# wkvong/multimodal-baby

Hardware: AMD Instinct MI355X
Metric: image-text pairs/sec, CVCL ResNeXt+embed 224², bs256, 1/2/4/8 MI355X (higher is better)
Workload: dtype bf16; 1 GPU; C2 = BASELINE configs[1]: CVCL saycam_contrastive, frozen random-init ResNeXt-50 32x4d (BN train mode) + embedding mean-pool text encoder, E=512, L2-normalised, fixed tau 0.07, 224x224 frames + 3-word utterances; full step = fwd + InfoNCE + bwd(fc, embedding) + AdamW; per_gpu_batch=256, global_batch=256, negatives=local (single GPU), parallelism=dp1, trunk_streams=2

## Files before the change

### include/cvcl_hip.h

```cpp
#ifndef CVCL_HIP_H
#define CVCL_HIP_H

#include <stddef.h>
#include <stdint.h>

#ifdef __cplusplus
extern "C" {
#endif

#define CVCL_ABI_VERSION 7

enum { CVCL_OK = 0, CVCL_EINVAL = -1, CVCL_ELAUNCH = -2, CVCL_EWORKSPACE = -3, CVCL_EUNSUPPORTED = -4 };
enum { CVCL_F32 = 0, CVCL_BF16 = 1, CVCL_F32X3 = 2 };
enum { CVCL_ACT_NONE = 0, CVCL_ACT_RELU = 1, CVCL_ACT_GELU = 2 };
#define CVCL_STATS_ACCUMULATE (-1)

int cvcl_abi_version(void);
const char* cvcl_last_error(void);

enum { CVCL_K_GEMM = 0, CVCL_K_GCONV = 1, CVCL_K_STEM = 2, CVCL_K_BN_FINALIZE = 3, CVCL_K_BN_ADD_RELU = 4,
       CVCL_K_MAXPOOL = 5, CVCL_K_AVGPOOL = 6, CVCL_K_HEAD = 7, CVCL_K_OTHER = 8, CVCL_K_ATTENTION = 9,
       CVCL_K_LAYERNORM = 10, CVCL_K_LSTM = 11, CVCL_K_GEMM_F32 = 12, CVCL_K_BN_APPLY = 13, CVCL_K_BN_BWD = 14,
       CVCL_K_WGRAD = 15, CVCL_K_GEMM8W = 16, CVCL_K_GEMM_PRO = 17, CVCL_K_NCLASSES = 18 };
int cvcl_prof_enable(int on);
// ... 48 lines not shown
int cvcl_gemm(int dtype, const cvcl_gemm_args* args, void* stream);
int cvcl_gemm_stats_rows(int dtype, const cvcl_gemm_args* args);
int cvcl_gemm8w(int epi, const cvcl_gemm_args* args, void* stream);
int cvcl_gemm_pro(const cvcl_gemm_args* args, void* stream);
int cvcl_gemm_pro_supported(const cvcl_gemm_args* args);
int cvcl_gemm_pro_stats_rows(int M, int N);
int cvcl_gemm8w_supported(int M, int N, int K, int lda, int ldw, int ldc);
int cvcl_set_gemm_cu_share(int cus);
int cvcl_gemm_ln_supported(const cvcl_gemm_args* args);
int cvcl_row_stats(int dtype, const void* x, long x_row_stride, float* out, long rows, int D, float eps, void* stream);
int cvcl_row_stats_finalize(const float* row_part, int strips, float* out, long rows, int D, float eps, void* stream);
int cvcl_gemm8w_tile_rows(int M, int N);
int cvcl_gemm8w_stats_rows(int M, int N);

size_t cvcl_conv1x1_gram_workspace_bytes(int K);
int cvcl_conv1x1_gram(const void* A, int lda, long M, int K, const float* a_scale, const float* a_shift, int a_relu, void* workspace,
                      size_t workspace_bytes, const double** gram_out, void* stream);
int cvcl_bn_from_gram(const double* gram, int K, long count, const void* W, int ldw, int N, const float* gamma, const float* beta,
                      float* running_mean, float* running_var, int64_t* num_batches_tracked, float momentum, float eps,
                      float* scale, float* shift, float* moments, int moments_ld, const float* centre, void* stream);

int cvcl_transpose_f32(const float* in, float* out, int rows, int cols, void* stream);
int cvcl_colsum_f32(const float* dY, float* d_bias, int M, int N, void* stream);

enum { CVCL_PACK_DENSE = 0, CVCL_PACK_STEM7 = 1, CVCL_PACK_GCONV3 = 2 };

typedef struct {
    const void* w;
    const float* gamma; const float* beta;
    float* running_mean; float* running_var; int64_t* num_batches_tracked;
} cvcl_convbn_params;

int cvcl_bn_finalize(const float* stats, int rows, long count, const float* gamma, const float* beta,
                     float* running_mean, float* running_var, int64_t* num_batches_tracked, float momentum,
                     float eps, float* scale, float* shift, const float* centre, int C, void* stream);
int cvcl_bn_eval_affine(const float* gamma, const float* beta, const float* running_mean, const float* running_var,
                        float eps, float* scale, float* shift, const float* centre, int C, void* stream);
int cvcl_col_stats_rows(long rows);
int cvcl_col_stats(int dtype, const void* x, long rows, int C, float* stats, int stats_rows, void* stream);

size_t cvcl_packed_weight_bytes(int dtype, int kind, int cout, int cin_per_group, int k);
int cvcl_pack_conv_weight(int dtype, int kind, const float* w_oihw, void* out, int cout, int cin_per_group, int k,
                          void* stream);

int cvcl_stem_conv_stats_rows(int dtype, int B, int H, int W);
int cvcl_stem_conv7x7(int dtype, const float* x_nchw, const void* w_packed, void* y_nhwc, float* stats, int stats_rows,
                      const float* centre , int B, int H, int W, void* stream);
int cvcl_stem_pool_supported(int dtype, int H, int W);
int cvcl_stem_pool(int dtype, const float* x_nchw, const void* w_packed, const float* scale, const float* shift,
                   const float* centre , void* y_nhwc, int B, int H, int W, void* stream);
int cvcl_bn_relu_maxpool(int dtype, const void* x, const float* scale, const float* shift, void* y, int B, int H, int W,
                         int C, void* stream);
int cvcl_gconv3x3_stats_rows(int dtype, int B, int H, int W, int C, int stride);
int cvcl_gconv3x3(int dtype, const void* x, const float* a_scale, const float* a_shift, const void* w_packed, void* y,
                  float* stats, int stats_rows, const float* centre , int B, int H, int W, int C, int groups,
                  int stride, void* stream);
int cvcl_bn_add_relu(int dtype, const void* raw, const float* scale, const float* shift, const void* idn,
                     const float* idn_scale, const float* idn_shift, void* out, long rows, int C, void* stream);
int cvcl_bn_relu_apply(int dtype, const void* x, const float* scale, const float* shift, void* y, long rows, int C,
                       void* stream);
int cvcl_avgpool(int dtype, const void* x, float* out, int B, int HW, int C, void* stream);

size_t cvcl_resnext50_workspace_bytes(int dtype, int B, int H, int W);
size_t cvcl_resnext50_centres_floats(void);
int cvcl_resnext50_fwd(int dtype, int B, int H, int W, int training, const float* x_nchw,
                       const cvcl_convbn_params* layers, int n_layers, void* workspace, size_t workspace_bytes,
                       void* layer4_out_nhwc, float* pooled, float momentum, float eps, const float* centres, void* stream);
size_t cvcl_resnext50_block_workspace_bytes(int dtype, int B, int h, int w, int stage);
int cvcl_resnext50_block_fwd(int dtype, int B, int h, int w, int stage, int first, int training, const void* x_nhwc,
                             const cvcl_convbn_params* layers, int n_layers, void* workspace, size_t workspace_bytes,
                             void* out_nhwc, float momentum, float eps, const float* centres ,
                             void* stream);
size_t cvcl_resnext50_moments_floats(void);
int cvcl_resnext50_fwd_deferred_stats(int dtype, int B, int H, int W, const float* x_nchw,
                                      const cvcl_convbn_params* layers, int n_layers, void* workspace, size_t workspace_bytes,
                                      void* layer4_out_nhwc, float* pooled, float eps, float* moments, const float* centres,
                                      void* stream);
int cvcl_resnext50_apply_moments(const cvcl_convbn_params* layers, int n_layers, const float* moments, float momentum,
                                 void* stream);
size_t cvcl_resnext50_fwd_grouped_workspace_bytes(int dtype, int B, int H, int W, int group);
int cvcl_resnext50_fwd_grouped(int dtype, int B, int H, int W, int group, const float* x_nchw,
                               const cvcl_convbn_params* layers, int n_layers, void* workspace, size_t workspace_bytes,
                               void* layer4_out_nhwc, float* pooled, float eps, void* stream);

int cvcl_im2col_patches(int dtype, const float* x_nchw, void* cols, int B, int H, int W, int patch, int Kpad,
                        void* stream);
int cvcl_vit_assemble_tokens(int dtype, const void* tok, const float* cls, const float* pos, void* h, int B, int T,
                             int D, void* stream);
int cvcl_layernorm(int dtype, const void* x, long x_row_stride, const float* gamma, const float* beta, float eps,
                   void* y, int y_is_f32, long rows, int D, void* stream);
int cvcl_attention(int dtype, const void* qkv, const int64_t* key_tok, void* out, int B, int T, int heads, int head_dim,
                   float scale, void* stream);
int cvcl_attention_mx(const void* qkv, void* out8, void* out_block_scales, int B, int T, int heads, int head_dim, float scale,
                      void* stream);
int cvcl_attention_train(const void* qkv, void* out, float* lse, int B, int T, int heads, int head_dim, float scale, void* stream);
int cvcl_attention_bwd(const void* qkv, const void* o, const void* d_o, const float* lse, void* d_qkv, int B, int T, int heads,
                       int head_dim, float scale, void* stream);
int cvcl_layernorm_bwd_rows_partials(long rows);
int cvcl_layernorm_bwd_rows(const void* x, long x_row_stride, const float* gamma, const void* dy, int dy_is_f32, long dy_row_stride,
                            float eps, const void* add, void* dx, long dx_row_stride, float* partial, long rows, int D, void* stream);
int cvcl_gelu_bf16(const void* u, const void* d_y, void* y, long n, void* stream);
int cvcl_vit_tokens_bwd(const void* dh, void* d_tok, float* d_pos, int B, int T, int D, void* stream);
int cvcl_attention_train_f32(const float* qkv, float* out, float* lse, int B, int T, int heads, int head_dim, float scale, void* stream);
int cvcl_attention_bwd_f32(const float* qkv, const float* o, const float* d_o, const float* lse, float* d_qkv, int B, int T, int heads,
                           int head_dim, float scale, void* stream);
int cvcl_layernorm_bwd_rows_f32(const float* x, long x_row_stride, const float* gamma, const float* dy, long dy_row_stride, float eps,
// ... 161 lines not shown
```

### multimodal-baby_amd/csrc/resnext.hip

```cpp
#include <algorithm>
#include <array>
#include <cstdlib>
#include <type_traits>

#include "cvcl_common.h"

namespace {

constexpr int kMaxStatsRows = 1024;
constexpr size_t kTrunkAccLayer = (size_t)kBnAccRows * 2 * 2048;


__global__ __launch_bounds__(1024) void bn_finalize_kernel(const float* __restrict__ stats, int rows, double count,
                                                           const float* __restrict__ gamma, const float* __restrict__ beta,
                                                           float* __restrict__ running_mean, float* __restrict__ running_var,
                                                           int64_t* __restrict__ nbt, float momentum, float eps,
                                                           float* __restrict__ scale, float* __restrict__ shift, int C,
                                                           float* __restrict__ moments, int moments_ld,
                                                           const float* __restrict__ centre) {
    constexpr int NS = 64, NC = 16;
    __shared__ double ps[NS][NC], pq[NS][NC];
    const int c = threadIdx.x & (NC - 1), sl = threadIdx.x / NC, ch = blockIdx.x * NC + c;
    double s = 0.0, q = 0.0;
    if (ch < C) {
// ... 519 lines not shown
        const int ox = (int)(p % Wo), oq = (int)((p / Wo) % Hq), b = (int)(p / ((long)Wo * Hq));
        const int oy = R * oq;
        float sc[8], sh[8], m[R][8];
#pragma unroll
        for (int e = 0; e < 8; ++e) {
            sc[e] = scale[cc * 8 + e]; sh[e] = shift[cc * 8 + e];
#pragma unroll
            for (int r = 0; r < R; ++r) m[r][e] = 0.f;
        }
        constexpr int EPC = ElemTraits<T>::kPerChunk, NC = 8 / EPC;
        Chunk<T> tap[NTAP][NC];
        const T* src[NTAP];
#pragma unroll
        for (int ky = 0; ky < NR; ++ky)
#pragma unroll
            for (int kx = 0; kx < 3; ++kx) {
                const int yin = min(max(2 * oy - 1 + ky, 0), H - 1);
                const int xin = min(max(2 * ox - 1 + kx, 0), W - 1);
                src[ky * 3 + kx] = x + (((long)b * H + yin) * W + xin) * C + cc * 8;
            }
        __builtin_amdgcn_sched_barrier(0);
#pragma unroll
        for (int t = 0; t < NTAP; ++t)
#pragma unroll
            for (int q = 0; q < NC; ++q) tap[t][q].load(src[t] + q * EPC);
        __builtin_amdgcn_sched_barrier(0);
#pragma unroll
        for (int t = 0; t < NTAP; ++t)
#pragma unroll
            for (int e = 0; e < 8; ++e) {
                const float v = fmaf(tap[t][e / EPC].get(e % EPC), sc[e], sh[e]);
#pragma unroll
                for (int r = 0; r < R; ++r)
                    if (t >= 6 * r && t < 6 * r + 9) m[r][e] = fmaxf(m[r][e], v);
            }
#pragma unroll
        for (int r = 0; r < R; ++r) {
            if (oy + r < Ho) {
                T* dst = y + (((long)b * Ho + oy + r) * Wo + ox) * C + cc * 8;
#pragma unroll
                for (int e = 0; e < 8; ++e) dst[e] = ElemTraits<T>::from_f(m[r][e]);
            }
        }
    }
}

constexpr int GC_CS = 64;
constexpr int GC_PIXB = 144;

struct GconvDev {
    const void* x; const float* a_scale; const float* a_shift; const void* w; void* y; float* stats;
    const float* centre;
    int B, H, W, C, cg, stride, Ho, Wo, TH, bands, rows_in;
    float act_floor;
    BnSrc src;
    int stats_acc;
};

template <bool WIDE, int NPF, int NMT>
__global__ __launch_bounds__(256, WIDE ? 2 : 3) void gconv_mfma_kernel(GconvDev p) {
    extern __shared__ __attribute__((aligned(16))) char smem[];
    const bf16_t* __restrict__ x = (const bf16_t*)p.x;
    bf16_t* __restrict__ y = (bf16_t*)p.y;
    const int tid = threadIdx.x, lane = tid & 63, wave = tid >> 6;
    const int pix = lane & 15, kb = lane >> 4;
    const int slab = blockIdx.y, c0 = slab * GC_CS;
    const int Wp = p.W + 2;
    constexpr bool wide = WIDE;
    constexpr int KS = WIDE ? 9 : 5;
    const int unit = c0 / 16 + wave;
    const bf16_t* wu = (const bf16_t*)p.w + (long)unit * KS * 512;
    bf16x8 wf[KS];
#pragma unroll
    for (int ks = 0; ks < KS; ++ks) wf[ks] = *reinterpret_cast<const bf16x8*>(wu + (ks * 16 + pix) * 32 + kb * 8);
    const int in_ch_off = wide ? ((wave >> 1) * 32 + kb * 8) : (wave * 16 + (kb & 1) * 8);

    const int s_chunk = tid & 7, s_pix0 = tid >> 3;
    f32x2 sc[4], sh[4];
    if (p.src.acc) {
        float* aff = reinterpret_cast<float*>(smem);
        bn_slice_affine<GC_CS>(p.src, c0, blockIdx.x == 0, aff, aff + 64);
#pragma unroll
        for (int e = 0; e < 4; ++e) {
            const int cl = s_chunk * 8 + 2 * e;
            sc[e] = f32x2{aff[cl], aff[cl + 1]};
            sh[e] = f32x2{aff[64 + cl], aff[64 + cl + 1]};
        }
        __syncthreads();
    } else {
#pragma unroll
        for (int e = 0; e < 4; ++e) {
            const int ch = c0 + s_chunk * 8 + 2 * e;
            sc[e] = p.a_scale ? f32x2{p.a_scale[ch], p.a_scale[ch + 1]} : f32x2{1.f, 1.f};
            sh[e] = p.a_scale ? f32x2{p.a_shift[ch], p.a_shift[ch + 1]} : f32x2{0.f, 0.f};
        }
    }
    const bool relu_in = p.act_floor == 0.f;
    f32x2 ssum[2] = {f32x2{0.f, 0.f}, f32x2{0.f, 0.f}}, ssq[2] = {f32x2{0.f, 0.f}, f32x2{0.f, 0.f}};

    const int npix_in = p.rows_in * Wp;
    const int n_out = p.TH * p.Wo, n_mt = cvcl_div_up(n_out, 16);
    int tap_off[KS];
#pragma unroll
    for (int ks = 0; ks < KS; ++ks) {
        int tap = wide ? ks : 2 * ks + (kb >> 1);
        if (tap > 8) tap = 8;
        const int ky = tap / 3, kx = tap - ky * 3;
        tap_off[ks] = (ky * Wp + kx) * GC_PIXB + in_ch_off * 2;
    }
    int mtab[NMT];
#pragma unroll
    for (int mt = 0; mt < NMT; ++mt) {
        const int q = pix + 16 * mt;
        const bool ok = mt < n_mt && q < n_out;
        const int ty = q / p.Wo, ox = q - ty * p.Wo;
        mtab[mt] = ok ? ((((ty * p.stride) * Wp + ox * p.stride) * GC_PIXB) | (ty << 16) | (1 << 24)) : 0;
    }
    char* s_out = smem + npix_in * GC_PIXB;
    u32x4 pf[NPF];
    bool pf_in[NPF];
    int slot_y[NPF], slot_xoff[NPF];
    bool slot_ok[NPF];
#pragma unroll
    for (int i = 0; i < NPF; ++i) {
        const int pi = s_pix0 + 32 * i;
        const int pc = min(pi, npix_in - 1);
        const int ry = pc / Wp, xin = pc - ry * Wp - 1;
        slot_y[i] = ry;
        slot_ok[i] = pi < npix_in && xin >= 0 && xin < p.W;
        slot_xoff[i] = min(max(xin, 0), p.W - 1) * p.C;
    }
    const int row_elems = p.W * p.C;
    auto prefetch = [&](int item) {
        const int b = item / p.bands, band = item - b * p.bands;
        const int iy0 = band * p.TH * p.stride - 1;
        const bf16_t* xb = x + (long)b * p.H * p.W * p.C + c0 + s_chunk * 8;
#pragma unroll
        for (int i = 0; i < NPF; ++i) {
            const int yin = iy0 + slot_y[i];
            pf_in[i] = slot_ok[i] && (unsigned)yin < (unsigned)p.H;
            const int yc = min(max(yin, 0), p.H - 1);
            pf[i] = *reinterpret_cast<const u32x4*>(xb + (yc * row_elems + slot_xoff[i]));
        }
    };
    f32x4 acc_init = {0.f, 0.f, 0.f, 0.f};
    if (p.centre) {
        const f32x4 cv = *reinterpret_cast<const f32x4*>(p.centre + c0 + wave * 16 + kb * 4);
        acc_init = f32x4{-cv[0], -cv[1], -cv[2], -cv[3]};
    }
    const int n_items = p.B * p.bands;
    const int st_off = (tid >> 3) * p.C + (tid & 7) * 8;
    __builtin_amdgcn_s_waitcnt(0x0F70);
    const int bx = (gridDim.x & 7) == 0 ? (int)((blockIdx.x & 7) * (gridDim.x >> 3) + (blockIdx.x >> 3)) : (int)blockIdx.x;
    if (bx < n_items) prefetch(bx);
    for (int item = bx; item < n_items; item += gridDim.x) {
        const int b = item / p.bands, band = item - b * p.bands;
        const int oy0 = band * p.TH;
        __syncthreads();
        auto stage = [&](auto RELU) __attribute__((always_inline)) {
#pragma unroll
            for (int i = 0; i < NPF; ++i) {
                const int pi = s_pix0 + 32 * i;
                const unsigned keep = pf_in[i] ? 0xffffffffu : 0u;
                u32x4 v;
#pragma unroll
                for (int e = 0; e < 4; ++e) {
                    unsigned y = round2(__builtin_elementwise_fma(widen2(pf[i][e]), sc[e], sh[e]));
                    if constexpr (decltype(RELU)::value) y = relu2(y);
                    v[e] = y & keep;
                }
                if (pi < npix_in) *reinterpret_cast<u32x4*>(smem + pi * GC_PIXB + s_chunk * 16) = v;
            }
        };
        if (relu_in) stage(std::true_type{});
        else stage(std::false_type{});
        __syncthreads();
        if (item + (int)gridDim.x < n_items) prefetch(item + gridDim.x);
        const int rows_left = p.Ho - oy0;
#pragma unroll
        for (int mt = 0; mt < NMT; mt += 2) {
            if (mt >= n_mt) break;
            const int e0 = mtab[mt], e1 = mtab[mt + 1];
            const int base0 = e0 & 0xffff, base1 = e1 & 0xffff;
            const int q0 = pix + 16 * mt, q1 = q0 + 16;
            const bool wr0 = (e0 >> 24) && ((e0 >> 16) & 0xff) < rows_left, wr1 = (e1 >> 24) && ((e1 >> 16) & 0xff) < rows_left;
            f32x4 acc0 = acc_init, acc1 = acc_init;
#pragma unroll
            for (int ks = 0; ks < KS; ++ks) {
                const bf16x8 a0 = *reinterpret_cast<const bf16x8*>(smem + base0 + tap_off[ks]);
                const bf16x8 a1 = *reinterpret_cast<const bf16x8*>(smem + base1 + tap_off[ks]);
                acc0 = __builtin_amdgcn_mfma_f32_16x16x32_bf16(wf[ks], a0, acc0, 0, 0, 0);
                acc1 = __builtin_amdgcn_mfma_f32_16x16x32_bf16(wf[ks], a1, acc1, 0, 0, 0);
            }
            if (wr0) {
                const u32x2 o = {round2(f32x2{acc0[0], acc0[1]}), round2(f32x2{acc0[2], acc0[3]})};
                *reinterpret_cast<u32x2*>(s_out + q0 * GC_PIXB + wave * 32 + kb * 8) = o;
#pragma unroll
                for (int e = 0; e < 2; ++e) { const f32x2 sv = widen2(o[e]); ssum[e] += sv; ssq[e] = __builtin_elementwise_fma(sv, sv, ssq[e]); }
            }
            if (wr1) {
                const u32x2 o = {round2(f32x2{acc1[0], acc1[1]}), round2(f32x2{acc1[2], acc1[3]})};
                *reinterpret_cast<u32x2*>(s_out + q1 * GC_PIXB + wave * 32 + kb * 8) = o;
#pragma unroll
                for (int e = 0; e < 2; ++e) { const f32x2 sv = widen2(o[e]); ssum[e] += sv; ssq[e] = __builtin_elementwise_fma(sv, sv, ssq[e]); }
            }
        }
        __syncthreads();
        const int valid_rows = min(p.TH, p.Ho - oy0);
        const int n_chunks = valid_rows * p.Wo * 8;
        bf16_t* yb = y + ((long)b * p.Ho + oy0) * p.Wo * p.C + c0 + st_off;
        const char* so = s_out + (tid >> 3) * GC_PIXB + (tid & 7) * 16;
#pragma unroll
        for (int k = 0; k < NMT / 2; ++k) {
            if (tid + 256 * k < n_chunks)
                *reinterpret_cast<bf16x8*>(yb + (long)k * 32 * p.C) = *reinterpret_cast<const bf16x8*>(so + k * 32 * GC_PIXB);
        }
    }
#pragma unroll
    for (int e = 0; e < 4; ++e) {
        float s = ssum[e >> 1][e & 1], q = ssq[e >> 1][e & 1];
#pragma unroll
        for (int o = 1; o < 16; o <<= 1) { s += __shfl_xor(s, o, 64); q += __shfl_xor(q, o, 64); }
        if (pix == 0 && p.stats) {
            const int ch = c0 + wave * 16 + kb * 4 + e;
            cvcl_bn_stats_out(p.stats, p.stats_acc, blockIdx.x, p.C, ch, s, q);
        }
    }
}

__global__ __launch_bounds__(256) void gconv_direct_f32_kernel(const float* __restrict__ x, const float* __restrict__ a_scale,
                                                               const float* __restrict__ a_shift, const float* __restrict__ w,
                                                               float* __restrict__ y, const float* __restrict__ centre,
                                                               int B, int H, int W, int C, int cg,
                                                               int stride, int Ho, int Wo, float act_floor) {
    const long total = (long)B * Ho * Wo * C;
    for (long i = (long)blockIdx.x * blockDim.x + threadIdx.x; i < total; i += (long)gridDim.x * blockDim.x) {
        const int co = (int)(i % C);
        const long pp = i / C;
        const int ox = (int)(pp % Wo), oy = (int)((pp / Wo) % Ho), b = (int)(pp / ((long)Wo * Ho));
        const int g0 = (co / cg) * cg;
        float acc = centre ? -centre[co] : 0.f;
        for (int ci = 0; ci < cg; ++ci) {
            const float sc = a_scale ? a_scale[g0 + ci] : 1.f, sh = a_scale ? a_shift[g0 + ci] : 0.f;
            for (int ky = 0; ky < 3; ++ky) {
                const int yin = oy * stride - 1 + ky;
                if (yin < 0 || yin >= H) continue;
                for (int kx = 0; kx < 3; ++kx) {
                    const int xin = ox * stride - 1 + kx;
                    if (xin < 0 || xin >= W) continue;
                    const float v = fmaxf(fmaf(x[(((long)b * H + yin) * W + xin) * C + g0 + ci], sc, sh), act_floor);
                    acc = fmaf(v, w[((long)co * cg + ci) * 9 + ky * 3 + kx], acc);
                }
            }
        }
        y[i] = acc;
    }
}

template <int CG>
__global__ __launch_bounds__(256) void gconv_tiled_f32_kernel(const float* __restrict__ x, const float* __restrict__ a_scale,
                                                              const float* __restrict__ a_shift, const float* __restrict__ w,
                                                              float* __restrict__ y, const float* __restrict__ centre,
                                                              int B, int H, int W, int C, int stride, int Ho, int Wo, int TH,
                                                              int bands, int plane_p, float act_floor) {
    extern __shared__ __attribute__((aligned(16))) float smf[];
    constexpr int NG = 64 / CG;
    const int Wp = W + 2, rows_in = (TH - 1) * stride + 3, plane = rows_in * Wp;
    float* ws = smf;
    float* cs = ws + 64 * 9 * CG;
// ... 459 lines not shown
        }
    }
    CVCL_LAUNCH_CHECK();
    if (stats) return cvcl_col_stats(CVCL_F32, y_nhwc, (long)B * (H / 2) * (W / 2), 64, stats, stats_rows, stream);
    return CVCL_OK;
}

extern "C" int cvcl_stem_pool_supported(int dtype, int H, int W) {
    return dtype == CVCL_BF16 && H % 2 == 0 && W % 4 == 0 && W / 4 <= 64 && W + 6 + 8 <= 2 * STEM_PITCH && W / 2 + 2 <= STEMP_BW;
}

extern "C" int cvcl_stem_pool(int dtype, const float* x_nchw, const void* w_packed, const float* scale, const float* shift,
                              const float* centre, void* y_nhwc, int B, int H, int W, void* stream) {
    CVCL_CHECK_DTYPE(dtype, "cvcl_stem_pool");
    CVCL_CHECK_ARG(x_nchw && w_packed && scale && shift && y_nhwc && B > 0, "cvcl_stem_pool: bad args");
    CVCL_CHECK_ARG(cvcl_stem_pool_supported(dtype, H, W), "cvcl_stem_pool: bf16 and a width <= %d only (got dtype %d, %d x %d)",
                   2 * (STEMP_BW - 2), dtype, H, W);
    const size_t lds = (size_t)3 * STEMP_ROWS * STEM_PITCH * 4 + (size_t)STEMP_CR * STEMP_BW * 128 + 3 * 64 * 4;
    static CvclLdsAttr attr;
    if (const int rc = cvcl_raise_lds_limit(attr, (const void*)stem_pool_mfma_kernel, (int)lds, "cvcl_stem_pool")) return rc;
    attr.mark();
    const int Hp = (H / 2 - 1) / 2 + 1;
    const int items = B * cvcl_div_up(Hp, STEMP_TP);
    int dev = 0, cus = 256;
    if (hipGetDevice(&dev) != hipSuccess || hipDeviceGetAttribute(&cus, hipDeviceAttributeMultiprocessorCount, dev) != hipSuccess || cus <= 0) cus = 256;
    const int grid = items < cus ? items : cus;
    CvclProfScope prof(stream, CVCL_K_STEM);
    hipLaunchKernelGGL(stem_pool_mfma_kernel, dim3(grid), dim3(512), lds, (hipStream_t)stream, x_nchw, (const bf16_t*)w_packed,
                       (bf16_t*)y_nhwc, scale, shift, centre, B, H, W);
    CVCL_LAUNCH_CHECK();
    return CVCL_OK;
}

extern "C" int cvcl_bn_relu_maxpool(int dtype, const void* x, const float* scale, const float* shift, void* y, int B,
                                    int H, int W, int C, void* stream) {
    CVCL_CHECK_DTYPE_TRUNK(dtype, "cvcl_bn_relu_maxpool");
    dtype = cvcl_storage_dtype(dtype);
    CVCL_CHECK_ARG(x && scale && shift && y && C % 8 == 0, "cvcl_bn_relu_maxpool: bad args");
    CvclProfScope prof(stream, CVCL_K_MAXPOOL);
    const int Ho = (H - 1) / 2 + 1, Wo = (W - 1) / 2 + 1;
    const long total = (long)B * ((Ho + POOL_ROWS - 1) / POOL_ROWS) * Wo * (C / 8);
    const int grid = cvcl_grid(total, 256, 8192);
    if (dtype == CVCL_F32)
        hipLaunchKernelGGL(bn_relu_maxpool_kernel<float>, dim3(grid), dim3(256), 0, (hipStream_t)stream,
                           (const float*)x, scale, shift, (float*)y, B, H, W, C);
    else
        hipLaunchKernelGGL(bn_relu_maxpool_kernel<bf16_t>, dim3(grid), dim3(256), 0, (hipStream_t)stream,
                           (const bf16_t*)x, scale, shift, (bf16_t*)y, B, H, W, C);
    CVCL_LAUNCH_CHECK();
    return CVCL_OK;
}

namespace {
struct GconvPlan { int TH, bands, rows_in, grid_x; size_t lds; };
GconvPlan gconv_plan(int B, int H, int W, int C, int stride) {
    GconvPlan g;
    const int Ho = (H - 1) / stride + 1, Wo = (W - 1) / stride + 1, Wp = W + 2;
    auto bytes = [&](int th) { return (size_t)(((th - 1) * stride + 3) * Wp + th * Wo) * GC_PIXB; };
    int TH = Ho;
    while (TH > 1 && (bytes(TH) > (size_t)52 * 1024 || ((TH - 1) * stride + 3) * Wp > 10 * 32 || TH * Wo > 128)) TH = (TH + 1) / 2;
    g.TH = TH;
    g.bands = cvcl_div_up(Ho, TH);
    g.rows_in = (TH - 1) * stride + 3;
    g.lds = bytes(TH);
    int per_cu = (int)((160 * 1024) / g.lds);
    const int reg_limit = (C / 32 == 32) ? 2 : 3;
    if (per_cu > reg_limit) per_cu = reg_limit;
    if (per_cu < 1) per_cu = 1;
    const int slabs = C / GC_CS;
    int gx = per_cu * 256 / slabs;
    if (gx < 1) gx = 1;
    const int items = B * g.bands;
    g.grid_x = items < gx ? items : gx;
    return g;
}
}

extern "C" int cvcl_gconv3x3_stats_rows(int dtype, int B, int H, int W, int C, int stride) {
    if (!cvcl_dtype_trunk(dtype)) return 0;
    if (dtype == CVCL_F32X3) return C % 32 == 0 ? cvcl_gconv_split_stats_rows(B, H, W, C, stride) : 0;
    if (dtype == CVCL_BF16) return gconv_plan(B, H, W, C, stride).grid_x;
    const int Ho = (H - 1) / stride + 1, Wo = (W - 1) / stride + 1;
    return cvcl_col_stats_rows((long)B * Ho * Wo);
}

static int gconv3x3_impl(int dtype, const void* x, const float* a_scale, const float* a_shift, const BnSrc* src, const void* w_packed,
                         void* y, float* stats, int stats_rows, const float* centre, int B, int H, int W, int C, int groups,
                         int stride, void* stream) {
    CVCL_CHECK_DTYPE_TRUNK(dtype, "cvcl_gconv3x3");
    CVCL_CHECK_ARG(x && w_packed && y && (!a_scale == !a_shift), "cvcl_gconv3x3: null pointer");
    CVCL_CHECK_ARG(!src || (dtype == CVCL_BF16 && src->acc && src->gamma && src->beta && src->C == C && src->count > 0 &&
                            (const void*)src->acc != (const void*)stats),
                   "cvcl_gconv3x3: finalize-on-load source");
    CVCL_CHECK_ARG(stats_rows != CVCL_STATS_ACCUMULATE || dtype == CVCL_BF16, "cvcl_gconv3x3: accumulators exist for bf16 only");
    const float act_floor = (a_scale || src) ? 0.f : -INFINITY;
    CVCL_CHECK_ARG(B > 0 && (stride == 1 || stride == 2) && groups > 0 && C % groups == 0, "cvcl_gconv3x3: bad shape");
    const int cg = C / groups;
    const int Ho = (H - 1) / stride + 1, Wo = (W - 1) / stride + 1;
    hipStream_t s = (hipStream_t)stream;
    if (dtype == CVCL_F32X3)
        return cvcl_gconv_split((const float*)x, a_scale, a_shift, act_floor, w_packed, (float*)y, stats, stats_rows, centre, B, H, W, C,
                                cg, stride, stream);
    if (dtype == CVCL_BF16) {
        CVCL_CHECK_ARG((cg == 4 || cg == 8 || cg == 16 || cg == 32) && C % GC_CS == 0,
                       "cvcl_gconv3x3: unsupported channels-per-group %d (C=%d)", cg, C);
        const GconvPlan g = gconv_plan(B, H, W, C, stride);
        CVCL_CHECK_ARG(g.lds <= 160 * 1024 && g.rows_in * (W + 2) <= 10 * 32 && g.TH * ((W - 1) / stride + 1) <= 128,
                       "cvcl_gconv3x3: feature map too wide for one staged band (%zu B, %d pixels)", g.lds, g.rows_in * (W + 2));
        CVCL_CHECK_ARG(!stats || stats_rows == CVCL_STATS_ACCUMULATE || stats_rows >= g.grid_x, "cvcl_gconv3x3: stats_rows %d < %d", stats_rows, g.grid_x);
        GconvDev d;
        d.x = x; d.a_scale = a_scale; d.a_shift = a_shift; d.w = w_packed; d.y = y; d.stats = stats; d.centre = centre;
        d.B = B; d.H = H; d.W = W; d.C = C; d.cg = cg; d.stride = stride; d.Ho = Ho; d.Wo = Wo;
        d.TH = g.TH; d.bands = g.bands; d.rows_in = g.rows_in;
        d.act_floor = act_floor;
        d.src = BnSrc{};
        d.stats_acc = stats && stats_rows == CVCL_STATS_ACCUMULATE;
        if (src) {
            CVCL_CHECK_ARG(g.lds >= 2048, "cvcl_gconv3x3: band buffers smaller than the finalize-on-load scratch");
            d.src = *src;
        }
        CvclProfScope prof(stream, CVCL_K_GCONV);
        int rc;
        const int slots = cvcl_div_up(g.rows_in * (W + 2), 32);
        static CvclLdsAttr attr_set[2][2][11];
        auto launch = [&](auto kern) -> int {
            CvclLdsAttr& done = attr_set[cg == 32][g.TH * Wo <= 64][slots <= 4 ? 4 : slots <= 6 ? 6 : slots <= 8 ? 8 : 10];
            if (const int rc = cvcl_raise_lds_limit(done, (const void*)kern, 160 * 1024, "cvcl_gconv3x3")) return rc;
            done.mark();
            hipLaunchKernelGGL(kern, dim3(g.grid_x, C / GC_CS), dim3(256), g.lds, s, d);
            return CVCL_OK;
        };
        const bool few = g.TH * Wo <= 64;
#define CVCL_GCONV_PICK(W_) \
        (slots <= 4 ? (few ? launch(gconv_mfma_kernel<W_, 4, 4>) : launch(gconv_mfma_kernel<W_, 4, 8>)) \
         : slots <= 6 ? (few ? launch(gconv_mfma_kernel<W_, 6, 4>) : launch(gconv_mfma_kernel<W_, 6, 8>)) \
         : slots <= 8 ? (few ? launch(gconv_mfma_kernel<W_, 8, 4>) : launch(gconv_mfma_kernel<W_, 8, 8>)) \
                      : (few ? launch(gconv_mfma_kernel<W_, 10, 4>) : launch(gconv_mfma_kernel<W_, 10, 8>)))
        rc = cg == 32 ? CVCL_GCONV_PICK(true) : CVCL_GCONV_PICK(false);
#undef CVCL_GCONV_PICK
        if (rc) return rc;
        CVCL_LAUNCH_CHECK();
        return CVCL_OK;
    }
    const long total = (long)B * Ho * Wo * C;
    {
        CvclProfScope prof(stream, CVCL_K_GCONV);
        auto plane_p_of = [&](int th) { const int pl = ((th - 1) * stride + 3) * (W + 2); return pl + ((9 - (pl & 7)) & 7); };
        auto lds_of = [&](int th) { return (size_t)(64 * 9 * cg + 64 + 64 * plane_p_of(th)) * 4; };
        int TH = Ho;
        while (TH > 1 && lds_of(TH) > 150 * 1024) --TH;
        const bool tiled = C % 64 == 0 && (cg == 4 || cg == 8 || cg == 16 || cg == 32) && lds_of(TH) <= 150 * 1024 &&
                           ((uintptr_t)x & 15) == 0 && ((uintptr_t)y & 15) == 0 && ((uintptr_t)a_scale & 15) == 0 && ((uintptr_t)a_shift & 15) == 0;
        if (tiled) {
            const int bands = cvcl_div_up(Ho, TH);
            const long items = (long)B * bands;
            const int slabs = C / 64;
            long gx = 1024 / slabs;
            if (gx < 1) gx = 1;
            if (gx > items) gx = items;
            static CvclLdsAttr attr[4];
            auto launch = [&](auto kern, int slot) -> int {
                if (const int rc = cvcl_raise_lds_limit(attr[slot], (const void*)kern, 160 * 1024, "cvcl_gconv3x3")) return rc;
                attr[slot].mark();
                hipLaunchKernelGGL(kern, dim3((unsigned)gx, slabs), dim3(256), lds_of(TH), s, (const float*)x, a_scale, a_shift,
                                   (const float*)w_packed, (float*)y, centre, B, H, W, C, stride, Ho, Wo, TH, bands, plane_p_of(TH), act_floor);
                return CVCL_OK;
            };
            const int rc = cg == 4 ? launch(gconv_tiled_f32_kernel<4>, 0) : cg == 8 ? launch(gconv_tiled_f32_kernel<8>, 1)
                         : cg == 16 ? launch(gconv_tiled_f32_kernel<16>, 2) : launch(gconv_tiled_f32_kernel<32>, 3);
            if (rc) return rc;
        } else {
            hipLaunchKernelGGL(gconv_direct_f32_kernel, dim3(cvcl_grid(total, 256, 8192)), dim3(256), 0, s, (const float*)x, a_scale,
                               a_shift, (const float*)w_packed, (float*)y, centre, B, H, W, C, cg, stride, Ho, Wo, act_floor);
        }
    }
    CVCL_LAUNCH_CHECK();
    if (stats) return cvcl_col_stats(CVCL_F32, y, (long)B * Ho * Wo, C, stats, stats_rows, stream);
    return CVCL_OK;
}

extern "C" int cvcl_gconv3x3(int dtype, const void* x, const float* a_scale, const float* a_shift, const void* w_packed,
                             void* y, float* stats, int stats_rows, const float* centre, int B, int H, int W, int C, int groups,
                             int stride, void* stream) {
    return gconv3x3_impl(dtype, x, a_scale, a_shift, nullptr, w_packed, y, stats, stats_rows, centre, B, H, W, C, groups, stride, stream);
}

extern "C" int cvcl_bn_add_relu(int dtype, const void* raw, const float* scale, const float* shift, const void* idn,
                                const float* idn_scale, const float* idn_shift, void* out, long rows, int C, void* stream) {
    CVCL_CHECK_DTYPE_TRUNK(dtype, "cvcl_bn_add_relu");
    dtype = cvcl_storage_dtype(dtype);
// ... 533 lines not shown
```

### multimodal-baby_amd/multimodal/_hip.py

```python
from __future__ import annotations

import ctypes as C
import os

import torch

_HERE = os.path.dirname(os.path.abspath(__file__))
LIB_PATH = os.path.join(os.path.dirname(_HERE), "lib", "libcvcl_hip.so")

F32, BF16, F32X3 = 0, 1, 2
ACT_NONE, ACT_RELU, ACT_GELU = 0, 1, 2
ABI_VERSION = 7
PACK_DENSE, PACK_STEM7, PACK_GCONV3 = 0, 1, 2
GRADCAM_ALL, GRADCAM_BLOCK_IMAGE, GRADCAM_BLOCK_TEXT = 0, 1, 2
FUSE_MEAN, FUSE_MAX, FUSE_MIN = 0, 1, 2
BEAM_MAX_K, BEAM_MAX_T = 16, 128
TOKEN_TOPK_MAX_K = 16
KERNEL_CLASSES = ("gemm", "gconv3x3", "stem7x7", "bn_finalize", "bn_add_relu", "bn_relu_maxpool", "avgpool", "head",
                  "other", "attention", "layernorm", "lstm", "gemm_f32", "bn_relu_apply", "bn_bwd", "wgrad", "gemm8w", "gemm_pro")


class CvclError(RuntimeError):
    pass

# ... 20 lines not shown

class GemmFp8Args(C.Structure):
    _fields_ = [
        ("A8", C.c_void_p), ("a_scale", C.c_void_p), ("a_block_scales", C.c_void_p), ("lda", C.c_int),
        ("W8", C.c_void_p), ("w_scale", C.c_void_p), ("ldw", C.c_int),
        ("C", C.c_void_p), ("ldc", C.c_int), ("c8", C.c_void_p), ("c_block_scales", C.c_void_p), ("ldc8", C.c_int),
        ("bias", C.c_void_p), ("act", C.c_int), ("R", C.c_void_p), ("ldr", C.c_int),
        ("M", C.c_int), ("N", C.c_int), ("K", C.c_int),
        ("ln_stats", C.c_void_p), ("ln_colsum", C.c_void_p), ("row_part", C.c_void_p),
    ]


class ConvBnParams(C.Structure):
    _fields_ = [("w", C.c_void_p), ("gamma", C.c_void_p), ("beta", C.c_void_p),
                ("running_mean", C.c_void_p), ("running_var", C.c_void_p), ("num_batches_tracked", C.c_void_p)]


_P, _I, _F, _SZ = C.c_void_p, C.c_int, C.c_float, C.c_size_t

SIGNATURES = {
    "cvcl_abi_version": (_I, []),
    "cvcl_last_error": (C.c_char_p, []),
    "cvcl_prof_enable": (_I, [_I]),
    "cvcl_prof_collect": (_I, [_P, _P, _I]),
    "cvcl_prof_null_bracket_us": (_I, [_P, _I, _P]),
    "cvcl_embed_meanpool_fwd": (_I, [_P, _P, _P, _P, _P, _I, _I, _I, _I, _P]),
    "cvcl_embed_meanpool_bwd": (_I, [_P, _P, _P, _P, _I, _I, _I, _I, _P]),
    "cvcl_l2norm_fwd": (_I, [_P, _P, _P, _I, _I, _F, _P]),
    "cvcl_l2norm_bwd": (_I, [_P, _P, _P, _P, _I, _I, _F, _P]),
    "cvcl_sim_logits_fwd": (_I, [_P, _P, _P, _P, _I, _I, _I, _P]),
    "cvcl_sim_logits_bwd_workspace_bytes": (_SZ, [_I, _I, _I]),
    "cvcl_sim_logits_bwd": (_I, [_P, _P, _P, _P, _P, _P, _P, _P, _I, _I, _I, _P, _SZ, _P]),
    "cvcl_sim_logits_bwd_rows": (_I, [_P, _P, _P, _P, _P, _P, _P, _P, _I, _I, _I, _I, _I, _I, _I, _P, _SZ, _P]),
    "cvcl_infonce_workspace_bytes": (_SZ, [_I]),
    "cvcl_infonce_fwd": (_I, [_P, _I, _P, _P, _P, _P, _SZ, _P]),
    "cvcl_infonce_bwd": (_I, [_P, _P, _P, _P, _P, _I, _P]),
    "cvcl_row_entropy": (_I, [_P, _P, _I, _I, _P]),
    "cvcl_gemm_grid_m": (_I, [_I, _I, _I, _I]),
    "cvcl_gemm": (_I, [_I, C.POINTER(GemmArgs), _P]),
    "cvcl_transpose_f32": (_I, [_P, _P, _I, _I, _P]),
    "cvcl_colsum_f32": (_I, [_P, _P, _I, _I, _P]),
    "cvcl_bn_finalize": (_I, [_P, _I, C.c_long, _P, _P, _P, _P, _P, _F, _F, _P, _P, _P, _I, _P]),
    "cvcl_bn_eval_affine": (_I, [_P, _P, _P, _P, _F, _P, _P, _P, _I, _P]),
    "cvcl_col_stats_rows": (_I, [C.c_long]),
    "cvcl_col_stats": (_I, [_I, _P, C.c_long, _I, _P, _I, _P]),
    "cvcl_packed_weight_bytes": (_SZ, [_I, _I, _I, _I, _I]),
    "cvcl_pack_conv_weight": (_I, [_I, _I, _P, _P, _I, _I, _I, _P]),
    "cvcl_stem_conv_stats_rows": (_I, [_I, _I, _I, _I]),
    "cvcl_stem_conv7x7": (_I, [_I, _P, _P, _P, _P, _I, _P, _I, _I, _I, _P]),
    "cvcl_stem_pool_supported": (_I, [_I, _I, _I]),
    "cvcl_stem_pool": (_I, [_I, _P, _P, _P, _P, _P, _P, _I, _I, _I, _P]),
    "cvcl_bn_relu_maxpool": (_I, [_I, _P, _P, _P, _P, _I, _I, _I, _I, _P]),
    "cvcl_gconv3x3_stats_rows": (_I, [_I, _I, _I, _I, _I, _I]),
    "cvcl_gconv3x3": (_I, [_I, _P, _P, _P, _P, _P, _P, _I, _P, _I, _I, _I, _I, _I, _I, _P]),
    "cvcl_bn_add_relu": (_I, [_I, _P, _P, _P, _P, _P, _P, _P, C.c_long, _I, _P]),
    "cvcl_bn_relu_apply": (_I, [_I, _P, _P, _P, _P, C.c_long, _I, _P]),
    "cvcl_avgpool": (_I, [_I, _P, _P, _I, _I, _I, _P]),
    "cvcl_im2col_patches": (_I, [_I, _P, _P, _I, _I, _I, _I, _I, _P]),
    "cvcl_vit_assemble_tokens": (_I, [_I, _P, _P, _P, _P, _I, _I, _I, _P]),
    "cvcl_layernorm": (_I, [_I, _P, C.c_long, _P, _P, _F, _P, _I, C.c_long, _I, _P]),
    "cvcl_attention": (_I, [_I, _P, _P, _P, _I, _I, _I, _I, _F, _P]),
    "cvcl_embed_gather_pos": (_I, [_P, _P, _P, _P, _I, _I, _I, _I, _P]),
    "cvcl_seq_sum_div": (_I, [_P, _P, _P, _I, _I, _I, _P]),
    "cvcl_lstm_cell": (_I, [_P, _P, _I, _P, _P, _P, _I, _I, _I, _P]),
    "cvcl_dropout": (_I, [_P, _P, _P, C.c_long, _F, C.c_ulonglong, C.c_long, C.c_long, _P]),
    "cvcl_layernorm_bwd": (_I, [_P, _P, _P, _F, _P, _P, C.c_long, _I, _P]),
    "cvcl_relu_bwd": (_I, [_P, _P, _P, C.c_long, _P]),
    "cvcl_embed_rows_bwd": (_I, [_P, _P, _P, _I, _I, _I, _P]),
    "cvcl_seq_sum_div_bwd": (_I, [_P, _P, _P, _I, _I, _I, _P]),
    "cvcl_attention_small": (_I, [_P, _P, _P, _P, _P, _I, _I, _I, _I, _F, _F, C.c_ulonglong, _P]),
    "cvcl_lstm_cell_train": (_I, [_P, _P, _I, _P, _P, _P, _P, _P, _P, _I, _I, _I, _P]),
    "cvcl_lstm_cell_bwd": (_I, [_P, _P, _P, _I, _P, _P, _P, _P, _I, _I, _I, _P]),
    "cvcl_bn_apply": (_I, [_I, _P, _P, _P, _P, C.c_long, _I, _I, _P]),
    "cvcl_bn_bwd_partial_rows": (_I, [_I, C.c_long, _I]),
    "cvcl_bn_bwd": (_I, [_I, _I, _P, _P, _P, _P, _P, _P, _P, _P, _P, _P, _P, _P, C.c_long, _I, _P, _I, _P, _P]),
    "cvcl_bn_batch_moments": (_I, [_P, _I, C.c_long, C.c_float, _P, _P, _P, _I, _P]),
    "cvcl_gconv_weight_dgrad": (_I, [_P, _P, _I, _I, _P]),
    "cvcl_transpose": (_I, [_I, _P, _P, C.c_long, _I, _P]),
    "cvcl_add": (_I, [_I, _P, _P, _P, C.c_long, _I, _P]),
    "cvcl_relu_mask": (_I, [_I, _P, _P, _P, C.c_long, _P]),
    "cvcl_maxpool3x3s2": (_I, [_I, _P, _P, _P, _I, _I, _I, _I, _P]),
    "cvcl_maxpool3x3s2_idx": (_I, [_I, _P, _P, _P, _P, _I, _I, _I, _I, _P]),
    "cvcl_avgpool_bwd": (_I, [_I, _P, _P, _I, _I, _I, _P]),
    "cvcl_zero_stuff2": (_I, [_I, _P, _P, _I, _I, _I, _I, _P]),
    "cvcl_conv_wgrad_direct": (_I, [_I, _P, _P, _P, _I, _I, _I, _I, _I, _I, _I, _I, _I, _I, _P]),
    "cvcl_gemm_tn_workspace_bytes": (C.c_size_t, [_I, C.c_long, _I, _I]),
    "cvcl_gemm_tn": (_I, [_I, _P, _I, _P, _I, C.c_long, _I, _I, _P, _I, _P, C.c_size_t, _P]),
    "cvcl_gconv3x3_wgrad_workspace_bytes": (C.c_size_t, [_I, _I, _I, _I, _I]),
    "cvcl_gconv3x3_wgrad": (_I, [_P, _P, _P, _I, _I, _I, _I, _I, _I, _P, C.c_size_t, _P]),
    "cvcl_stem_im2col": (_I, [_P, _P, _I, _I, _I, _P]),
    "cvcl_gemm_stats_rows": (_I, [_I, _P]),
    "cvcl_gemm_pro": (_I, [_P, _P]),
    "cvcl_gemm_pro_supported": (_I, [_P]),
    "cvcl_gemm_pro_stats_rows": (_I, [_I, _I]),
    "cvcl_gemm8w": (_I, [_I, _P, _P]),
    "cvcl_gemm8w_supported": (_I, [_I, _I, _I, _I, _I, _I]),
    "cvcl_gemm_ln_supported": (_I, [C.POINTER(GemmArgs)]),
    "cvcl_set_gemm_cu_share": (_I, [_I]),
    "cvcl_conv1x1_gram_workspace_bytes": (C.c_size_t, [_I]),
    "cvcl_conv1x1_gram": (_I, [_P, _I, C.c_long, _I, _P, _P, _I, _P, C.c_size_t, C.POINTER(C.c_void_p), _P]),
    "cvcl_bn_from_gram": (_I, [_P, _I, C.c_long, _P, _I, _I, _P, _P, _P, _P, _P, _F, _F, _P, _P, _P, _I, _P, _P]),
    "cvcl_row_stats": (_I, [_I, _P, C.c_long, _P, C.c_long, _I, _F, _P]),
    "cvcl_row_stats_finalize": (_I, [_P, _I, _P, C.c_long, _I, _F, _P]),
    "cvcl_gemm8w_tile_rows": (_I, [_I, _I]),
    "cvcl_gemm8w_stats_rows": (_I, [_I, _I]),
    "cvcl_bf16_to_f32": (_I, [_P, _P, C.c_long, _P]),
# ... 298 lines not shown
```

Baseline: 51460 pairs/s.

## Reuse overlapping halo rows across consecutive bands in grouped 3x3 conv

Each block in the grouped 3x3 MFMA conv now processes a contiguous run of bands within an image rather than striding across the grid. When the new rows per band cover the halo, it copies the overlapping input rows already held in LDS to the head of the buffer instead of re-reading and re-normalising them from global memory. The grid is capped at half the item count so runs have length at least two. This cuts global reads and BN-apply work on halo rows, at the cost of an extra LDS copy plus barrier, more registers (new template variants, lower occupancy for large halos), and possible load imbalance from contiguous work assignment.

Measured after the change: 51640 pairs/s, median of 4. Within noise of the previous version (+0.4%).

```diff
diff --git a/include/cvcl_hip.h b/include/cvcl_hip.h
--- a/include/cvcl_hip.h
+++ b/include/cvcl_hip.h
@@ -124,6 +124,7 @@
 int cvcl_bn_relu_maxpool(int dtype, const void* x, const float* scale, const float* shift, void* y, int B, int H, int W,
                          int C, void* stream);
 int cvcl_gconv3x3_stats_rows(int dtype, int B, int H, int W, int C, int stride);
+int cvcl_gconv3x3_run_length(int dtype, int B, int H, int W, int C, int stride);
 int cvcl_gconv3x3(int dtype, const void* x, const float* a_scale, const float* a_shift, const void* w_packed, void* y,
                   float* stats, int stats_rows, const float* centre , int B, int H, int W, int C, int groups,
                   int stride, void* stream);
diff --git a/multimodal-baby_amd/csrc/resnext.hip b/multimodal-baby_amd/csrc/resnext.hip
--- a/multimodal-baby_amd/csrc/resnext.hip
+++ b/multimodal-baby_amd/csrc/resnext.hip
@@ -595,13 +595,14 @@
     const void* x; const float* a_scale; const float* a_shift; const void* w; void* y; float* stats;
     const float* centre;
     int B, H, W, C, cg, stride, Ho, Wo, TH, bands, rows_in;
+    int carry;
     float act_floor;
     BnSrc src;
     int stats_acc;
 };
 
-template <bool WIDE, int NPF, int NMT>
-__global__ __launch_bounds__(256, WIDE ? 2 : 3) void gconv_mfma_kernel(GconvDev p) {
+template <bool WIDE, int NPF, int NHD, int NMT>
+__global__ __launch_bounds__(256, (WIDE || NPF + NHD > 12) ? 2 : 3) void gconv_mfma_kernel(GconvDev p) {
     extern __shared__ __attribute__((aligned(16))) char smem[];
     const bf16_t* __restrict__ x = (const bf16_t*)p.x;
     bf16_t* __restrict__ y = (bf16_t*)p.y;
@@ -641,7 +642,7 @@
     const bool relu_in = p.act_floor == 0.f;
     f32x2 ssum[2] = {f32x2{0.f, 0.f}, f32x2{0.f, 0.f}}, ssq[2] = {f32x2{0.f, 0.f}, f32x2{0.f, 0.f}};
 
-    const int npix_in = p.rows_in * Wp;
+    const int npix_in = p.rows_in * Wp, npix_new = p.TH * p.stride * Wp, npix_head = npix_in - npix_new;
     const int n_out = p.TH * p.Wo, n_mt = cvcl_div_up(n_out, 16);
     int tap_off[KS];
 #pragma unroll
@@ -660,24 +661,44 @@
         mtab[mt] = ok ? ((((ty * p.stride) * Wp + ox * p.stride) * GC_PIXB) | (ty << 16) | (1 << 24)) : 0;
     }
     char* s_out = smem + npix_in * GC_PIXB;
-    u32x4 pf[NPF];
-    bool pf_in[NPF];
-    int slot_y[NPF], slot_xoff[NPF];
-    bool slot_ok[NPF];
-#pragma unroll
-    for (int i = 0; i < NPF; ++i) {
-        const int pi = s_pix0 + 32 * i;
-        const int pc = min(pi, npix_in - 1);
+    u32x4 pf[NPF], hd[NHD];
+    bool pf_in[NPF], hd_in[NHD];
+    int slot_y[NPF], slot_xoff[NPF], head_pk[NHD];
+    bool slot_ok[NPF], head_ok[NHD];
+    auto slot_of = [&](int pi, int npix, int row0, int& sy, int& sx, bool& ok) {
+        const int pc = min(pi, npix - 1);
         const int ry = pc / Wp, xin = pc - ry * Wp - 1;
-        slot_y[i] = ry;
-        slot_ok[i] = pi < npix_in && xin >= 0 && xin < p.W;
-        slot_xoff[i] = min(max(xin, 0), p.W - 1) * p.C;
+        sy = row0 + ry;
+        ok = pi < npix && xin >= 0 && xin < p.W;
+        sx = min(max(xin, 0), p.W - 1) * p.C;
+    };
+#pragma unroll
+    for (int i = 0; i < NPF; ++i) slot_of(s_pix0 + 32 * i, npix_new, p.rows_in - p.TH * p.stride, slot_y[i], slot_xoff[i], slot_ok[i]);
+#pragma unroll
+    for (int i = 0; i < NHD; ++i) {
+        int hy, hx;
+        slot_of(s_pix0 + 32 * i, npix_head, 0, hy, hx, head_ok[i]);
+        head_pk[i] = hx | (hy << 28);
     }
     const int row_elems = p.W * p.C;
-    auto prefetch = [&](int item) {
-        const int b = item / p.bands, band = item - b * p.bands;
+    const int n_items = p.B * p.bands;
+    const int bx = (gridDim.x & 7) == 0 ? (int)((blockIdx.x & 7) * (gridDim.x >> 3) + (blockIdx.x >> 3)) : (int)blockIdx.x;
+    const int run_len = n_items / (int)gridDim.x, run_rem = n_items - run_len * (int)gridDim.x;
+    const int it0 = bx * run_len + min(bx, run_rem), it1 = it0 + run_len + (bx < run_rem);
+    auto prefetch = [&](int b, int band, bool first) {
         const int iy0 = band * p.TH * p.stride - 1;
         const bf16_t* xb = x + (long)b * p.H * p.W * p.C + c0 + s_chunk * 8;
+        if (first) {
+#pragma unroll
+            for (int i = 0; i < NHD; ++i) {
+                int pk = head_pk[i];
+                asm volatile("" : "+v"(pk));
+                const int yin = iy0 + (pk >> 28);
+                hd_in[i] = head_ok[i] && (unsigned)yin < (unsigned)p.H;
+                const int yc = min(max(yin, 0), p.H - 1);
+                hd[i] = *reinterpret_cast<const u32x4*>(xb + (yc * row_elems + (pk & 0x0fffffff)));
+            }
+        }
 #pragma unroll
         for (int i = 0; i < NPF; ++i) {
             const int yin = iy0 + slot_y[i];
@@ -691,34 +712,48 @@
         const f32x4 cv = *reinterpret_cast<const f32x4*>(p.centre + c0 + wave * 16 + kb * 4);
         acc_init = f32x4{-cv[0], -cv[1], -cv[2], -cv[3]};
     }
-    const int n_items = p.B * p.bands;
     const int st_off = (tid >> 3) * p.C + (tid & 7) * 8;
     __builtin_amdgcn_s_waitcnt(0x0F70);
-    const int bx = (gridDim.x & 7) == 0 ? (int)((blockIdx.x & 7) * (gridDim.x >> 3) + (blockIdx.x >> 3)) : (int)blockIdx.x;
-    if (bx < n_items) prefetch(bx);
-    for (int item = bx; item < n_items; item += gridDim.x) {
-        const int b = item / p.bands, band = item - b * p.bands;
+    int b = it0 / p.bands, band = it0 - b * p.bands;
+    bool first = true;
+    prefetch(b, band, first);
+    for (int item = it0; item < it1; ++item) {
         const int oy0 = band * p.TH;
+        const bool more = item + 1 < it1, wrap = band + 1 == p.bands;
+        const int b_next = wrap ? b + 1 : b, band_next = wrap ? 0 : band + 1;
+        const bool first_next = wrap || !p.carry;
         __syncthreads();
         auto stage = [&](auto RELU) __attribute__((always_inline)) {
-#pragma unroll
-            for (int i = 0; i < NPF; ++i) {
-                const int pi = s_pix0 + 32 * i;
-                const unsigned keep = pf_in[i] ? 0xffffffffu : 0u;
+            auto act = [&](const u32x4& raw, bool in) {
+                const unsigned keep = in ? 0xffffffffu : 0u;
                 u32x4 v;
 #pragma unroll
                 for (int e = 0; e < 4; ++e) {
-                    unsigned y = round2(__builtin_elementwise_fma(widen2(pf[i][e]), sc[e], sh[e]));
+                    unsigned y = round2(__builtin_elementwise_fma(widen2(raw[e]), sc[e], sh[e]));
                     if constexpr (decltype(RELU)::value) y = relu2(y);
                     v[e] = y & keep;
                 }
-                if (pi < npix_in) *reinterpret_cast<u32x4*>(smem + pi * GC_PIXB + s_chunk * 16) = v;
+                return v;
+            };
+            if (first) {
+#pragma unroll
+                for (int i = 0; i < NHD; ++i) {
+                    const int pi = s_pix0 + 32 * i;
+                    const u32x4 v = act(hd[i], hd_in[i]);
+                    if (pi < npix_head) *reinterpret_cast<u32x4*>(smem + pi * GC_PIXB + s_chunk * 16) = v;
+                }
+            }
+#pragma unroll
+            for (int i = 0; i < NPF; ++i) {
+                const int pi = s_pix0 + 32 * i;
+                const u32x4 v = act(pf[i], pf_in[i]);
+                if (pi < npix_new) *reinterpret_cast<u32x4*>(smem + (npix_head + pi) * GC_PIXB + s_chunk * 16) = v;
             }
         };
         if (relu_in) stage(std::true_type{});
         else stage(std::false_type{});
         __syncthreads();
-        if (item + (int)gridDim.x < n_items) prefetch(item + gridDim.x);
+        if (more) prefetch(b_next, band_next, first_next);
         const int rows_left = p.Ho - oy0;
 #pragma unroll
         for (int mt = 0; mt < NMT; mt += 2) {
@@ -749,6 +784,15 @@
             }
         }
         __syncthreads();
+        if (more && !first_next) {
+            u32x4 t[NHD];
+#pragma unroll
+            for (int i = 0; i < NHD; ++i)
+                t[i] = *reinterpret_cast<const u32x4*>(smem + (npix_new + min(s_pix0 + 32 * i, npix_head - 1)) * GC_PIXB + s_chunk * 16);
+#pragma unroll
+            for (int i = 0; i < NHD; ++i)
+                if (s_pix0 + 32 * i < npix_head) *reinterpret_cast<u32x4*>(smem + (s_pix0 + 32 * i) * GC_PIXB + s_chunk * 16) = t[i];
+        }
         const int valid_rows = min(p.TH, p.Ho - oy0);
         const int n_chunks = valid_rows * p.Wo * 8;
         bf16_t* yb = y + ((long)b * p.Ho + oy0) * p.Wo * p.C + c0 + st_off;
@@ -758,6 +802,7 @@
             if (tid + 256 * k < n_chunks)
                 *reinterpret_cast<bf16x8*>(yb + (long)k * 32 * p.C) = *reinterpret_cast<const bf16x8*>(so + k * 32 * GC_PIXB);
         }
+        b = b_next; band = band_next; first = first_next;
     }
 #pragma unroll
     for (int e = 0; e < 4; ++e) {
@@ -1323,7 +1368,7 @@
 }
 
 namespace {
-struct GconvPlan { int TH, bands, rows_in, grid_x; size_t lds; };
+struct GconvPlan { int TH, bands, rows_in, grid_x, carry, run; size_t lds; };
 GconvPlan gconv_plan(int B, int H, int W, int C, int stride) {
     GconvPlan g;
     const int Ho = (H - 1) / stride + 1, Wo = (W - 1) / stride + 1, Wp = W + 2;
@@ -1335,16 +1380,24 @@
     g.rows_in = (TH - 1) * stride + 3;
     g.lds = bytes(TH);
     int per_cu = (int)((160 * 1024) / g.lds);
-    const int reg_limit = (C / 32 == 32) ? 2 : 3;
+    const int reg_limit = (C / 32 == 32 || cvcl_div_up(TH * stride * Wp, 32) > 8 || cvcl_div_up((g.rows_in - TH * stride) * Wp, 32) > 4) ? 2 : 3;
     if (per_cu > reg_limit) per_cu = reg_limit;
     if (per_cu < 1) per_cu = 1;
     const int slabs = C / GC_CS;
     int gx = per_cu * 256 / slabs;
     if (gx < 1) gx = 1;
     const int items = B * g.bands;
+    g.carry = g.bands > 1 && TH * stride >= g.rows_in - TH * stride;
+    if (g.carry && gx > items / 2) gx = items / 2;
     g.grid_x = items < gx ? items : gx;
+    g.run = g.carry ? (items / g.grid_x < g.bands ? items / g.grid_x : g.bands) : 1;
     return g;
 }
+}
+
+extern "C" int cvcl_gconv3x3_run_length(int dtype, int B, int H, int W, int C, int stride) {
+    if (dtype != CVCL_BF16 || B <= 0 || H <= 0 || W <= 0 || C <= 0 || C % GC_CS || (stride != 1 && stride != 2)) return 0;
+    return gconv_plan(B, H, W, C, stride).run;
 }
 
 extern "C" int cvcl_gconv3x3_stats_rows(int dtype, int B, int H, int W, int C, int stride) {
@@ -1378,11 +1431,12 @@
         const GconvPlan g = gconv_plan(B, H, W, C, stride);
         CVCL_CHECK_ARG(g.lds <= 160 * 1024 && g.rows_in * (W + 2) <= 10 * 32 && g.TH * ((W - 1) / stride + 1) <= 128,
                        "cvcl_gconv3x3: feature map too wide for one staged band (%zu B, %d pixels)", g.lds, g.rows_in * (W + 2));
+        CVCL_CHECK_ARG((long)W * C < (1L << 28), "cvcl_gconv3x3: input row of %ld elements", (long)W * C);
         CVCL_CHECK_ARG(!stats || stats_rows == CVCL_STATS_ACCUMULATE || stats_rows >= g.grid_x, "cvcl_gconv3x3: stats_rows %d < %d", stats_rows, g.grid_x);
         GconvDev d;
         d.x = x; d.a_scale = a_scale; d.a_shift = a_shift; d.w = w_packed; d.y = y; d.stats = stats; d.centre = centre;
         d.B = B; d.H = H; d.W = W; d.C = C; d.cg = cg; d.stride = stride; d.Ho = Ho; d.Wo = Wo;
-        d.TH = g.TH; d.bands = g.bands; d.rows_in = g.rows_in;
+        d.TH = g.TH; d.bands = g.bands; d.rows_in = g.rows_in; d.carry = g.carry;
         d.act_floor = act_floor;
         d.src = BnSrc{};
         d.stats_acc = stats && stats_rows == CVCL_STATS_ACCUMULATE;
@@ -1392,10 +1446,11 @@
         }
         CvclProfScope prof(stream, CVCL_K_GCONV);
         int rc;
-        const int slots = cvcl_div_up(g.rows_in * (W + 2), 32);
-        static CvclLdsAttr attr_set[2][2][11];
+        const int s_new = cvcl_div_up(g.TH * stride * (W + 2), 32), s_head = cvcl_div_up((g.rows_in - g.TH * stride) * (W + 2), 32);
+        const int pick = s_new <= 4 && s_head <= 2 ? 0 : s_new <= 4 && s_head <= 4 ? 1 : s_new <= 8 && s_head <= 2 ? 2 : 3;
+        static CvclLdsAttr attr_set[2][2][4];
         auto launch = [&](auto kern) -> int {
-            CvclLdsAttr& done = attr_set[cg == 32][g.TH * Wo <= 64][slots <= 4 ? 4 : slots <= 6 ? 6 : slots <= 8 ? 8 : 10];
+            CvclLdsAttr& done = attr_set[cg == 32][g.TH * Wo <= 64][pick];
             if (const int rc = cvcl_raise_lds_limit(done, (const void*)kern, 160 * 1024, "cvcl_gconv3x3")) return rc;
             done.mark();
             hipLaunchKernelGGL(kern, dim3(g.grid_x, C / GC_CS), dim3(256), g.lds, s, d);
@@ -1403,10 +1458,10 @@
         };
         const bool few = g.TH * Wo <= 64;
 #define CVCL_GCONV_PICK(W_) \
-        (slots <= 4 ? (few ? launch(gconv_mfma_kernel<W_, 4, 4>) : launch(gconv_mfma_kernel<W_, 4, 8>)) \
-         : slots <= 6 ? (few ? launch(gconv_mfma_kernel<W_, 6, 4>) : launch(gconv_mfma_kernel<W_, 6, 8>)) \
-         : slots <= 8 ? (few ? launch(gconv_mfma_kernel<W_, 8, 4>) : launch(gconv_mfma_kernel<W_, 8, 8>)) \
-                      : (few ? launch(gconv_mfma_kernel<W_, 10, 4>) : launch(gconv_mfma_kernel<W_, 10, 8>)))
+        (pick == 0 ? (few ? launch(gconv_mfma_kernel<W_, 4, 2, 4>) : launch(gconv_mfma_kernel<W_, 4, 2, 8>)) \
+         : pick == 1 ? (few ? launch(gconv_mfma_kernel<W_, 4, 4, 4>) : launch(gconv_mfma_kernel<W_, 4, 4, 8>)) \
+         : pick == 2 ? (few ? launch(gconv_mfma_kernel<W_, 8, 2, 4>) : launch(gconv_mfma_kernel<W_, 8, 2, 8>)) \
+                     : (few ? launch(gconv_mfma_kernel<W_, 10, 8, 4>) : launch(gconv_mfma_kernel<W_, 10, 8, 8>)))
         rc = cg == 32 ? CVCL_GCONV_PICK(true) : CVCL_GCONV_PICK(false);
 #undef CVCL_GCONV_PICK
         if (rc) return rc;
diff --git a/multimodal-baby_amd/multimodal/_hip.py b/multimodal-baby_amd/multimodal/_hip.py
--- a/multimodal-baby_amd/multimodal/_hip.py
+++ b/multimodal-baby_amd/multimodal/_hip.py
@@ -96,6 +96,7 @@
     "cvcl_stem_pool": (_I, [_I, _P, _P, _P, _P, _P, _P, _I, _I, _I, _P]),
     "cvcl_bn_relu_maxpool": (_I, [_I, _P, _P, _P, _P, _I, _I, _I, _I, _P]),
     "cvcl_gconv3x3_stats_rows": (_I, [_I, _I, _I, _I, _I, _I]),
+    "cvcl_gconv3x3_run_length": (_I, [_I, _I, _I, _I, _I, _I]),
     "cvcl_gconv3x3": (_I, [_I, _P, _P, _P, _P, _P, _P, _I, _P, _I, _I, _I, _I, _I, _I, _P]),
     "cvcl_bn_add_relu": (_I, [_I, _P, _P, _P, _P, _P, _P, _P, C.c_long, _I, _P]),
     "cvcl_bn_relu_apply": (_I, [_I, _P, _P, _P, _P, C.c_long, _I, _P]),
```
